# Sbte/RAILS

Measured on AMD Instinct MI355X. Metric: RAILS iterations/sec (+ A*V SpMM HBM GB/s in roofline), m=1M rows/GPU, k=128, fp64, higher is better.
Workload: dtype f64

## Files before the change

include/rails_hip.h:

```cpp
#ifndef RAILS_HIP_H
#define RAILS_HIP_H

#include <stddef.h>
#include <stdint.h>

#ifdef __cplusplus
extern "C" {
#endif

#define RAILS_OK 0
#define RAILS_EINVAL -1
#define RAILS_EHIP -2
#define RAILS_ENOMEM -3
#define RAILS_ELAPACK -4
#define RAILS_ECOMM -5
#define RAILS_ENODEV -6

typedef struct rails_ctx rails_ctx;
typedef struct rails_csr rails_csr;
typedef struct rails_panel rails_panel;

const char *rails_last_error(void);
const char *rails_version(void);

// ... 123 lines not shown
int rails_sweep_plan_array(const rails_sweep_plan *plan, int which, const void **ptr, int64_t *count);


int rails_panel_create(rails_ctx *ctx, int64_t m_local, int capacity, rails_panel **out);
int rails_panel_create_ld(rails_ctx *ctx, int64_t m_local, int capacity, int ld, rails_panel **out);
int rails_panel_destroy(rails_panel *P);
int64_t rails_panel_rows(const rails_panel *P);
int rails_panel_capacity(const rails_panel *P);
int rails_panel_ld(const rails_panel *P);
void *rails_panel_device_ptr(const rails_panel *P);
int rails_panel_reserve(rails_ctx *ctx, rails_panel *P, int capacity);

int rails_panel_upload(rails_ctx *ctx, rails_panel *P, int c0, int nc, const double *host, int64_t ldh);
int rails_panel_download(rails_ctx *ctx, const rails_panel *P, int c0, int nc, double *host, int64_t ldh);

int rails_panel_fill(rails_ctx *ctx, rails_panel *P, int c0, int nc, double value);
int rails_panel_scale(rails_ctx *ctx, rails_panel *P, int c0, int nc, double s);
int rails_panel_copy(rails_ctx *ctx, const rails_panel *X, int xc0, int nc, rails_panel *Y, int yc0);
int rails_panel_axpy(rails_ctx *ctx, double alpha, const rails_panel *X, int xc0, int nc, rails_panel *Y,
                     int yc0);
int rails_panel_random(rails_ctx *ctx, rails_panel *P, int c0, int nc);

int rails_gram(rails_ctx *ctx, const rails_panel *X, int xc0, int a, const rails_panel *Y, int yc0, int b,
               double *C_host, int ldc);

int rails_panel_gemm(rails_ctx *ctx, double alpha, const rails_panel *X, int xc0, int k, const double *C_host,
                     int ldc, int r, double beta, rails_panel *Y, int yc0);

int rails_ctx_enable_library_gemm(rails_ctx *ctx);
int rails_ctx_library_gemm_ready(const rails_ctx *ctx);

int rails_deferred_reserve(rails_ctx *ctx, int nslots, int64_t doubles_per_slot);
int rails_gram_deferred(rails_ctx *ctx, const rails_panel *X, int xc0, int a, const rails_panel *Y, int yc0, int b, int slot);
int rails_panel_gemm_deferred(rails_ctx *ctx, double alpha, const rails_panel *X, int xc0, int k, int slot, int ld, int r, double beta,
                              rails_panel *Y, int yc0);
int rails_chol_inverse_deferred(rails_ctx *ctx, int slot_in, int w, int slot_out);
int rails_update_gram_deferred(rails_ctx *ctx, double alpha, const rails_panel *X, int xc0, int k, const double *C_host, int ldc, int r,
                               rails_panel *Y, int yc0, int r2, int slot);
int rails_update_gram_deferred_out(rails_ctx *ctx, double alpha, const rails_panel *X, int xc0, int k, const double *C_host, int ldc, int r,
                                   const rails_panel *Y, int yc0, rails_panel *Yout, int oc0, int r2, int slot);
int rails_deferred_fetch(rails_ctx *ctx, int slot, int64_t n, double *host_out);

int rails_panel_gemm_wide(rails_ctx *ctx, double alpha, const rails_panel *X, int xc0, int k, const double *C_host, int ldc, int r,
                          double beta, rails_panel *Y, int yc0);

void rails_dense_set_tile_fit(int on);
int rails_dense_tile_fit(void);
int rails_dense_last_tiles(const rails_ctx *ctx, int *update_gram_nbw, int *gram_cols_ti, int *gemm_wide_tr);

void rails_dense_set_update_gram_pipeline(int on);
int rails_dense_update_gram_pipeline(void);
int rails_dense_last_update_gram_form(const rails_ctx *ctx, int *form);

int rails_orthogonalize(rails_ctx *ctx, rails_panel *V, int k_old, int w, int method, int *used);
int rails_orthogonalize_deflated(rails_ctx *ctx, rails_panel *V, int k_old, int w, const rails_panel *N, int nc0, int q, int method, int *used);

int rails_panel_colnorms2(rails_ctx *ctx, const rails_panel *X, int c0, int nc, double *out_host);

int rails_orthogonalize_range(rails_ctx *ctx, rails_panel *V, int k_old, int w, const rails_panel *N, int nc0, int q, double tol, int *kept,
                              int32_t *kept_idx);

int rails_resid_lanczos(rails_ctx *ctx, const rails_panel *AV, int avc0, const rails_panel *MV, int mvc0, int k,
                        const double *T_host, int ldt, const rails_panel *B, int bc0, int p, int L,
                        double *H_host, int ldh, int *steps);

int rails_resid_lanczos_sparse(rails_ctx *ctx, const rails_panel *AV, int avc0, const rails_panel *MV, int mvc0, int k, const double *T_host,
                               int ldt, const rails_sprhs *S, int L, double *H_host, int ldh, int *steps);

int rails_lanczos_start(rails_ctx *ctx, const rails_panel *AV, int avc0, const rails_panel *MV, int mvc0, int k,
                        const rails_panel *B, int bc0, int p, double *sums_host);

int rails_lanczos_vectors(rails_ctx *ctx, const double *S_host, int lds, int w, rails_panel *Out, int oc0);
int rails_lanczos_last_launch(rails_ctx *ctx, int *nch, int *unroll, int *nblocks);
int rails_lanczos_release(rails_ctx *ctx);

int rails_ctx_reserve_staging(rails_ctx *ctx, size_t bytes);
int rails_timer_start(rails_ctx *ctx);
int rails_timer_stop(rails_ctx *ctx, double *ms);


void rails_sb03md(char dico, char job, char fact, char trans, int n, double *A, int lda, double *X, int ldx,
                  double *scale, int *info);
void rails_sb03md_counts(long *smith, long *schur);
void rails_sb03md_adi_counts(long *extended, long *fresh);
void rails_sb03md_set_pause(int calls);
void rails_dsyev(char jobz, char uplo, int n, double *a, int lda, double *w, int *info);
void rails_dsteqr(char compz, int n, double *d, double *e, double *z, int ldz, double *work, int *info);
void rails_dgemm(char transa, char transb, int m, int n, int k, double alpha, const double *A, int lda, const double *B,
                 int ldb, double beta, double *C, int ldc);
void rails_dtrsm(char side, char uplo, char transa, char diag, int m, int n, double alpha, const double *A, int lda, double *B, int ldb);
void rails_dpotrf(char uplo, int n, double *a, int lda, int *info);
void rails_dpstrf(char uplo, int n, double *a, int lda, int *piv, int *rank, double tol, int *info);
void rails_range_basis(int m, int n, double *a, int lda, double tol, double *q, int ldq, int *rank, int *info);
int rails_host_lapack_init(const char *path);
const char *rails_host_lapack_path(void);

#ifdef __cplusplus
}
#endif
#endif
```

rails_amd/_lib.py:

```python
import ctypes as C
import os

_HERE = os.path.dirname(os.path.abspath(__file__))
LIB_PATH = os.path.join(_HERE, "lib", "librails_hip.so")

_dp = C.POINTER(C.c_double)
_ip = C.POINTER(C.c_int)
_i64p = C.POINTER(C.c_int64)
_i32p = C.POINTER(C.c_int32)
_vp = C.c_void_p

ALLREDUCE_FN = C.CFUNCTYPE(C.c_int, C.c_void_p, C.c_void_p, C.c_size_t, C.c_void_p)
HALO_FN = C.CFUNCTYPE(C.c_int, C.c_void_p, C.c_void_p, C.c_void_p, C.c_int, C.c_void_p)
APPLY_FN = C.CFUNCTYPE(C.c_int, C.c_void_p, C.c_int, C.c_void_p, C.c_int, C.c_int, C.c_void_p, C.c_int)

SIGNATURES = {
    "rails_last_error": (C.c_char_p, []),
    "rails_version": (C.c_char_p, []),
    "rails_ctx_create": (C.c_int, [C.c_int, _vp, C.POINTER(_vp)]),
    "rails_ctx_destroy": (C.c_int, [_vp]),
    "rails_ctx_sync": (C.c_int, [_vp]),
    "rails_ctx_stream": (_vp, [_vp]),
    "rails_ctx_num_cu": (C.c_int, [_vp]),
    "rails_ctx_set_meter": (C.c_int, [_vp, C.c_int]),
# ... 53 lines not shown
    "rails_sptrsv_levels": (C.c_int64, [_vp]),
    "rails_sptrsv_solve": (C.c_int, [_vp, _vp, _vp, C.c_int, C.c_int]),
    "rails_panel_permute_rows": (C.c_int, [_vp, _vp, C.c_int, C.c_int, _vp, C.c_int, _vp, C.c_int]),
    "rails_index_upload": (C.c_int, [_vp, _i32p, C.c_int64, C.POINTER(_vp)]),
    "rails_index_free": (None, [_vp, _vp]),
    "rails_lu_create": (C.c_int, [_vp, C.c_int64, _i64p, _i32p, _dp, _i64p, _i32p, _dp, _i32p, _i32p, _i32p, C.c_int64, C.POINTER(_vp)]),
    "rails_lu_destroy": (None, [_vp]),
    "rails_lu_solve": (C.c_int, [_vp, _vp, C.c_int, _vp, C.c_int, C.c_int, _vp, C.c_int]),
    "rails_lu_stats": (C.c_int, [_vp, _i64p, C.c_int]),
    "rails_csr_create_lu": (C.c_int, [_vp, _vp, C.POINTER(_vp)]),
    "rails_iter_create": (C.c_int, [_vp, _vp, C.c_int, _dp, C.POINTER(_vp)]),
    "rails_iter_set": (C.c_int, [_vp, C.c_char_p, C.c_double]),
    "rails_iter_solve": (C.c_int, [_vp, _vp, C.c_int, _vp, C.c_int, C.c_int, _vp, C.c_int]),
    "rails_iter_precondition": (C.c_int, [_vp, _vp, _vp, C.c_int, C.c_int, _vp, C.c_int]),
    "rails_iter_amg_setup": (C.c_int, [_vp, _vp]),
    "rails_iter_amg_info": (C.c_int, [_vp, _i64p, _i64p, _dp, C.c_int]),
    "rails_iter_block_amg_setup": (C.c_int, [_vp, _vp]),
    "rails_iter_block_amg_info": (C.c_int, [_vp, _i64p, _i64p, _dp, C.c_int]),
    "rails_iter_block_jacobi": (C.c_int, [_vp, _vp, C.c_int, _dp]),
    "rails_iter_block_jacobi_info": (C.c_int64, [_vp, _ip, _dp, C.c_int64]),
    "rails_iter_stats": (C.c_int, [_vp, _dp, C.c_int]),
    "rails_iter_columns": (C.c_int, [_vp, _i32p, _dp, _i32p, C.c_int]),
    "rails_csr_create_iter": (C.c_int, [_vp, _vp, C.POINTER(_vp)]),
    "rails_iter_destroy": (None, [_vp]),
    "rails_csr_transpose_host": (C.c_int, [C.c_int64, C.c_int64, _i64p, _i32p, _dp, _i64p, _i32p, _dp]),
    "rails_csr_gram_norm2_host": (C.c_int, [C.c_int64, C.c_int64, _i64p, _i32p, _dp, _i64p, _i32p, _dp, _dp]),
    "rails_bsr_count_host": (C.c_int, [C.c_int64, C.c_int64, C.c_int, _i64p, _i32p, _i64p]),
    "rails_bsr_fill_host": (C.c_int, [C.c_int64, C.c_int64, C.c_int, _i64p, _i32p, _dp, _i64p, _i32p, _dp]),
    "rails_bsr_transpose_host": (C.c_int, [C.c_int64, C.c_int64, C.c_int, _i64p, _i32p, _dp, _i64p, _i32p, _dp]),
    "rails_csr_create_bsr": (C.c_int, [_vp, C.c_int64, C.c_int64, C.c_int, _i64p, _i32p, _dp, C.POINTER(_vp)]),
    "rails_csr_block_size": (C.c_int, [_vp]),
    "rails_csr_bsr_stats": (C.c_int, [_vp, _i64p, C.c_int]),
    "rails_sprhs_create": (C.c_int, [_vp, C.c_int64, C.c_int, _i64p, _i32p, _dp, C.POINTER(_vp)]),
    "rails_sprhs_destroy": (None, [_vp]),
    "rails_sprhs_rows": (C.c_int64, [_vp]),
    "rails_sprhs_cols": (C.c_int64, [_vp]),
    "rails_sprhs_nnz": (C.c_int64, [_vp]),
    "rails_sprhs_gram_norm2": (C.c_double, [_vp]),
    "rails_sprhs_apply": (C.c_int, [_vp, _vp, C.c_int, _vp, C.c_int, C.c_int, _vp, C.c_int]),
    "rails_csr_create_sprhs": (C.c_int, [_vp, _vp, C.POINTER(_vp)]),
    "rails_csr_cols": (C.c_int64, [_vp]),
    "rails_csr_sprhs": (_vp, [_vp]),
    "rails_resid_lanczos_sparse": (C.c_int, [_vp, _vp, C.c_int, _vp, C.c_int, C.c_int, _dp, C.c_int, _vp, C.c_int, _dp, C.c_int, _ip]),
    "rails_panel_random": (C.c_int, [_vp, _vp, C.c_int, C.c_int]),
    "rails_gram": (C.c_int, [_vp, _vp, C.c_int, C.c_int, _vp, C.c_int, C.c_int, _dp, C.c_int]),
    "rails_panel_gemm": (C.c_int, [_vp, C.c_double, _vp, C.c_int, C.c_int, _dp, C.c_int, C.c_int, C.c_double, _vp, C.c_int]),
    "rails_panel_gemm_wide": (C.c_int, [_vp, C.c_double, _vp, C.c_int, C.c_int, _dp, C.c_int, C.c_int, C.c_double, _vp, C.c_int]),
    "rails_dense_set_tile_fit": (None, [C.c_int]),
    "rails_dense_tile_fit": (C.c_int, []),
    "rails_dense_last_tiles": (C.c_int, [_vp, _ip, _ip, _ip]),
    "rails_dense_set_update_gram_pipeline": (None, [C.c_int]),
    "rails_dense_update_gram_pipeline": (C.c_int, []),
    "rails_dense_last_update_gram_form": (C.c_int, [_vp, _ip]),
    "rails_orthogonalize": (C.c_int, [_vp, _vp, C.c_int, C.c_int, C.c_int, _ip]),
    "rails_orthogonalize_deflated": (C.c_int, [_vp, _vp, C.c_int, C.c_int, _vp, C.c_int, C.c_int, C.c_int, _ip]),
    "rails_panel_colnorms2": (C.c_int, [_vp, _vp, C.c_int, C.c_int, _dp]),
    "rails_orthogonalize_range": (C.c_int, [_vp, _vp, C.c_int, C.c_int, _vp, C.c_int, C.c_int, C.c_double, _ip, _i32p]),
    "rails_resid_lanczos": (C.c_int, [_vp, _vp, C.c_int, _vp, C.c_int, C.c_int, _dp, C.c_int, _vp, C.c_int, C.c_int, C.c_int,
                                      _dp, C.c_int, _ip]),
    "rails_lanczos_start": (C.c_int, [_vp, _vp, C.c_int, _vp, C.c_int, C.c_int, _vp, C.c_int, C.c_int, _dp]),
    "rails_lanczos_vectors": (C.c_int, [_vp, _dp, C.c_int, C.c_int, _vp, C.c_int]),
    "rails_lanczos_last_launch": (C.c_int, [_vp, _ip, _ip, _ip]),
    "rails_lanczos_release": (C.c_int, [_vp]),
    "rails_timer_start": (C.c_int, [_vp]),
    "rails_timer_stop": (C.c_int, [_vp, _dp]),
    "rails_sb03md": (None, [C.c_char, C.c_char, C.c_char, C.c_char, C.c_int, _dp, C.c_int, _dp, C.c_int, _dp, _ip]),
    "rails_dsyev": (None, [C.c_char, C.c_char, C.c_int, _dp, C.c_int, _dp, _ip]),
    "rails_dsteqr": (None, [C.c_char, C.c_int, _dp, _dp, _dp, C.c_int, _dp, _ip]),
    "rails_ctx_reserve_staging": (C.c_int, [_vp, C.c_size_t]),
    "rails_sb03md_set_pause": (None, [C.c_int]),
    "rails_sb03md_counts": (None, [C.POINTER(C.c_long), C.POINTER(C.c_long)]),
    "rails_sb03md_adi_counts": (None, [C.POINTER(C.c_long), C.POINTER(C.c_long)]),
    "rails_dtrsm": (None, [C.c_char, C.c_char, C.c_char, C.c_char, C.c_int, C.c_int, C.c_double, _dp, C.c_int, _dp, C.c_int]),
    "rails_dgemm": (None, [C.c_char, C.c_char, C.c_int, C.c_int, C.c_int, C.c_double, _dp, C.c_int, _dp, C.c_int, C.c_double, _dp, C.c_int]),
    "rails_dpotrf": (None, [C.c_char, C.c_int, _dp, C.c_int, _ip]),
    "rails_dpstrf": (None, [C.c_char, C.c_int, _dp, C.c_int, _ip, _ip, C.c_double, _ip]),
    "rails_range_basis": (None, [C.c_int, C.c_int, _dp, C.c_int, C.c_double, _dp, C.c_int, _ip, _ip]),
    "rails_host_lapack_init": (C.c_int, [C.c_char_p]),
    "rails_host_lapack_path": (C.c_char_p, []),
}

_lib = None


class RailsError(RuntimeError):
    pass


def load():
    global _lib
    if _lib is not None:
        return _lib
    if not os.path.exists(LIB_PATH):
        raise RailsError(
            "rails_amd: %s is missing -- build it with `python -c 'import __graft_entry__ as g; g.build()'` "
            "or `make -C rails_amd/csrc`; there is no CPU fallback" % LIB_PATH)
    lib = C.CDLL(LIB_PATH, mode=C.RTLD_GLOBAL)
    for name, (res, args) in SIGNATURES.items():
        fn = getattr(lib, name)
        fn.restype = res
        fn.argtypes = args
    try:
        from ._solver_sigs import bind as _bind_solver
        _bind_solver(lib)
    except ImportError:
        pass
# ... 12 lines not shown
```

rails_amd/csrc/dense_choice.h:

```cpp
#pragma once
#include <algorithm>
#include <cstddef>
#include <cstdint>

namespace dense {

struct DenseSwitches {
    bool tile_fit = true;
    bool update_gram_pipeline = true;
    int gram_cols = 1;
    int gram_extra_column = 1;
    int fused_update_gram = 1;
    int panel_gemm_wide = 1;
    int num_cu = 256;
};

constexpr int inst(int a, int b = 0, int c = 0) { return (a << 16) | (b << 8) | c; }

inline bool rows_vec_ok(const void *ptr, int ld) { return (((uintptr_t)ptr) & 15) == 0 && (ld % 2) == 0; }

#define RAILS_DENSE_GRAM_TABLE(X) X(1, 1) X(8, 1) X(1, 8) X(2, 2) X(4, 2) X(2, 4)
#define RAILS_DENSE_GRAM2_TABLE(X) X(1, 1) X(8, 1) X(4, 2)
#define RAILS_DENSE_GRAM_COLS_TABLE(X) X(4, 1, 0) X(5, 1, 0) X(6, 1, 0) X(4, 1, 1) X(5, 1, 1) X(6, 1, 1) X(3, 2, 0) X(4, 2, 0) X(5, 2, 0)

enum class GramForm { RowSplit, WideX };
struct GramChoice {
    GramForm form;
    int ti, tj, ne;
    int64_t nslab, rps;
    int ngj;
    unsigned grid_y;
    int key() const { return form == GramForm::WideX ? inst(ti, tj, ne) : inst(ti, tj); }
};

inline void gram_slabs(int64_t m, int a, int b, int64_t *nslab_out, int64_t *rps_out)
{
    double bound = 0.02 * (double)m * (double)(a + b) / ((double)a * (double)b);
    int64_t nslab = (int64_t)std::min<double>(1024.0, std::max<double>(1.0, bound));
    int64_t maxslab = (m + 15) / 16;
    if (nslab > maxslab) nslab = std::max<int64_t>(1, maxslab);
    int64_t rps = (m + nslab - 1) / nslab;
    rps = (rps + 15) / 16 * 16;
    if (rps < 16) rps = 16;
    *nslab_out = std::max<int64_t>(1, (m + rps - 1) / rps);
    *rps_out = rps;
}

inline int gram_cols_tiles(int ntiles, bool one_tile, bool tile_fit)
{
    const int cand2[3] = {3, 4, 5}, cand1[3] = {4, 6, 8};
    const int *cand = one_tile ? cand1 : cand2;
    int best = cand[1], best_cost = 1 << 30;
    for (int q = 0; q < 3; ++q) {
        int ti = cand[q], strips = (ntiles + ti - 1) / ti, cost = (strips + 3) / 4 * 4 * ti;
        if (cost < best_cost) best = ti, best_cost = cost;
    }
    if (one_tile && best == 6 && (ntiles + 4) / 5 == (ntiles + 5) / 6 && tile_fit) best = 5;
    return best;
}

inline bool gram_wide_shape(int a, int b) { return b <= 32 && a >= 128; }

inline GramChoice gram_choice(int64_t m, int a, int b, bool two_segment, const DenseSwitches &sw)
{
    GramChoice g{};
    gram_slabs(m, a, b, &g.nslab, &g.rps);
// ... 35 lines not shown
    int64_t ntiles;
    int key() const { return inst(nbw, ne); }
};

inline UpdateGramChoice update_gram_choice(int64_t m, int k, int r, int r2, bool rows_ok, const DenseSwitches &sw)
{
    UpdateGramChoice u{};
    u.fused = sw.fused_update_gram && rows_ok && r <= 17 && r2 <= 16 && k >= 32 && k <= 512 && m >= 4096;
    if (!u.fused) return u;
    u.pipelined = sw.update_gram_pipeline;
    u.ntiles = (m + 15) / 16;
    u.grid = (unsigned)std::min<int64_t>(u.ntiles, 2 * (int64_t)std::max(sw.num_cu, 1));
    u.ne = r > 16 ? 1 : 0;
    if (k <= 256)
        u.nbw = 4;
    else if (k <= 320 && sw.tile_fit)
        u.nbw = 5;
    else if (k <= 384)
        u.nbw = 6;
    else
        u.nbw = 8;
    return u;
}

#define RAILS_DENSE_PANEL_GEMM_TABLE(X) X(1, 32) X(2, 32) X(4, 32) X(8, 32) X(16, 16)
#define RAILS_DENSE_PANEL_GEMM2_TABLE(X) X(1, 32) X(2, 32)

struct PanelGemmChoice {
    int tr, kc;
    int key() const { return inst(tr, kc); }
};

inline PanelGemmChoice panel_gemm_choice(int r)
{
    const int tiles = (r + 15) / 16;
    if (tiles <= 1) return {1, 32};
    if (tiles <= 2) return {2, 32};
    if (tiles <= 4) return {4, 32};
    if (tiles <= 8) return {8, 32};
    return {16, 16};
}
inline PanelGemmChoice panel_gemm2_choice(int r) { return {r <= 16 ? 1 : 2, 32}; }

#define RAILS_DENSE_GEMM_WIDE_TABLE(X) X(6) X(8) X(10) X(12) X(13) X(14) X(15) X(16) X(17) X(18)

struct GemmWideSlice {
    int j0, nc, tr;
};
struct GemmWidePlan {
    bool own_kernel;
    bool tile_fit;
    int r, nslices, width;
    size_t ct_doubles;
    int count() const { return own_kernel ? (r + width - 1) / width : 0; }
    GemmWideSlice slice(int j) const
    {
        const int j0 = j * width, nc = std::min(width, r - j0), exact = (nc + 15) / 16;
        const int tr = (tile_fit && (exact == 13 || exact == 15 || exact == 17)) ? exact : (nc + 31) / 32 * 2;
        return {j0, nc, tr < 6 ? 6 : tr > 18 ? 18 : tr};
    }
};

inline GemmWidePlan gemm_wide_plan(int k, int r, const DenseSwitches &sw)
{
    GemmWidePlan p{};
    p.own_kernel = sw.panel_gemm_wide && r > 64 && k >= 32;
    p.tile_fit = sw.tile_fit;
    p.r = r;
    if (!p.own_kernel) return p;
    p.nslices = (r + 287) / 288;
    p.width = ((r + p.nslices - 1) / p.nslices + 15) / 16 * 16;
    p.ct_doubles = (size_t)((k + 31) / 32 * 32) * (16 * 18 + 4);
    return p;
}

struct Inst {
    int a, b, c;
};
#define RAILS_DENSE_INST2(A, B) {A, B, 0},
#define RAILS_DENSE_INST3(A, B, C) {A, B, C},
#define RAILS_DENSE_INST1(A) {A, 0, 0},
constexpr Inst kGram[] = {RAILS_DENSE_GRAM_TABLE(RAILS_DENSE_INST2)};
constexpr Inst kGram2[] = {RAILS_DENSE_GRAM2_TABLE(RAILS_DENSE_INST2)};
constexpr Inst kGramCols[] = {RAILS_DENSE_GRAM_COLS_TABLE(RAILS_DENSE_INST3)};
constexpr Inst kUpdateGram[] = {RAILS_DENSE_UPDATE_GRAM_TABLE(RAILS_DENSE_INST2)};
constexpr Inst kPanelGemm[] = {RAILS_DENSE_PANEL_GEMM_TABLE(RAILS_DENSE_INST2)};
constexpr Inst kPanelGemm2[] = {RAILS_DENSE_PANEL_GEMM2_TABLE(RAILS_DENSE_INST2)};
constexpr Inst kGemmWide[] = {RAILS_DENSE_GEMM_WIDE_TABLE(RAILS_DENSE_INST1)};
#undef RAILS_DENSE_INST1
#undef RAILS_DENSE_INST2
#undef RAILS_DENSE_INST3

}
```

rails_amd/csrc/dense_common.h:

```cpp
#pragma once
#include "rails_internal.h"

#include <algorithm>
#include <atomic>

#include "dense_choice.h"

struct DenseSwitch {
    const char *variable;
    int on_by_default;
    std::atomic<int> v{-1};
    bool get()
    {
        if (v.load(std::memory_order_relaxed) < 0) {
            const char *e = getenv(variable);
            int undecided = -1;
            v.compare_exchange_strong(undecided, (e ? atoi(e) : on_by_default) ? 1 : 0);
        }
        return v.load(std::memory_order_relaxed) != 0;
    }
    void set(int on) { v.store(on ? 1 : 0); }
};
extern DenseSwitch g_dense_tile_fit;
extern DenseSwitch g_dense_update_gram_pipeline;

int rails_reduce_partials(rails_ctx *c, const double *partial, int64_t nslab, int64_t n, double *out);

inline int upload_coefficients(rails_ctx *c, const double *C_host, int ldc, int k, int r)
{
    const size_t n = (size_t)k * r;
    RAILS_TRY(rails_small_reserve(c, n * sizeof(double)));
    RAILS_TRY(rails_pinned_begin_write(c, n * sizeof(double)));
    for (int j = 0; j < r; ++j) memcpy(c->pinned + (size_t)j * k, C_host + (size_t)j * ldc, sizeof(double) * k);
    RAILS_HIP_CHECK(hipMemcpyAsync(c->small, c->pinned, n * sizeof(double), hipMemcpyHostToDevice, c->stream));
    return rails_pinned_end_write(c);
}

namespace {

typedef double v4f64 __attribute__((ext_vector_type(4)));
typedef double v2f64 __attribute__((ext_vector_type(2)));

__device__ __forceinline__ v4f64 mfma_f64(double a, double b, v4f64 c)
{
    return __builtin_amdgcn_mfma_f64_16x16x4f64(a, b, c, 0, 0, 0);
}

struct OneSeg {
    const double *X;
    int ld;
    struct Row {
        const double *x;
    };
    __device__ int col(int c) const { return c; }
    __device__ Row row(int64_t r) const { return {X + r * ld}; }
    __device__ static const double *at(Row r, int c) { return r.x + c; }
};
struct TwoSeg {
    const double *X1;
    int ld1, a1;
    const double *X2;
    int ld2;
    struct Col {
        int off;
        bool second;
    };
    struct Row {
        const double *x1, *x2;
    };
    __device__ Col col(int c) const
    {
        const bool second = c >= a1;
        return {second ? c - a1 : c, second};
    }
    __device__ Row row(int64_t r) const { return {X1 + r * ld1, X2 + r * ld2}; }
    __device__ static const double *at(Row r, Col c) { return (c.second ? r.x2 : r.x1) + c.off; }
};
// ... 3 lines not shown
```

rails_amd/csrc/dense_gemm.hip:

```cpp
#include "dense_common.h"

#include <dlfcn.h>
#include <mutex>

namespace {

template <int TR, int KC>
__global__ __launch_bounds__(256) void k_panel_gemm(double alpha, const double *X, int ldx, int k,
                                                    const double *__restrict__ C, int r, double beta, double *Yp,
                                                    int ldy, int64_t m, int vec_ok)
{
    const OneSeg Xo{X, ldx};
#define RAILS_PG_VEC4(c) (vec_ok && (c) + 4 <= k)
#include "dense_panel_gemm.inc"
}

template <int TR, int KC>
__global__ __launch_bounds__(256) void k_panel_gemm2(double alpha, const double *X1, int ldx1, int a1, const double *X2, int ldx2, int a,
                                                     const double *__restrict__ C, int r, double beta, double *Yp, int ldy, int64_t m, int vec1,
                                                     int vec2)
{
    const TwoSeg Xo{X1, ldx1, a1, X2, ldx2};
    const int k = a;
#define RAILS_PG_VEC4(c) (((c) + 4 <= a1 && vec1) || ((c) >= a1 && (c) + 4 <= a && vec2))
// ... 52 lines not shown
        }
    };
    double xa[4], xb[4];
    stage(0);
    fetch(4 * kk, xa);
    fetch(16 + 4 * kk, xb);
    asm volatile("s_waitcnt vmcnt(0)" : : : "memory");
    __builtin_amdgcn_s_barrier();
    for (int ci = 0; ci < nchunks; ++ci) {
        if (ci + 1 < nchunks) stage(ci + 1);
        double xc[4], xd[4];
        fetch((ci + 1) * KC + 4 * kk, xc);
        fetch((ci + 1) * KC + 16 + 4 * kk, xd);
        const double *cb = Cs + (size_t)(ci & 1) * (KC * RL);
#pragma unroll
        for (int s = 0; s < 4; ++s) {
            const double *crow = &cb[(4 * kk + s) * RL + li];
#pragma unroll
            for (int t = 0; t < TR; ++t) acc[t] = mfma_f64(xa[s], crow[16 * t], acc[t]);
        }
        if (!skip_tail || ci * KC + 16 < k) {
#pragma unroll
            for (int s = 0; s < 4; ++s) {
                const double *crow = &cb[(16 + 4 * kk + s) * RL + li];
#pragma unroll
                for (int t = 0; t < TR; ++t) acc[t] = mfma_f64(xb[s], crow[16 * t], acc[t]);
            }
        }
#pragma unroll
        for (int s = 0; s < 4; ++s) {
            xa[s] = xc[s];
            xb[s] = xd[s];
        }
        asm volatile("s_waitcnt vmcnt(0) lgkmcnt(0)" : : : "memory");
        __builtin_amdgcn_s_barrier();
    }
#pragma unroll
    for (int t = 0; t < TR; ++t) {
        const int j = 16 * t + li;
        if (j >= r) continue;
#pragma unroll
        for (int v = 0; v < 4; ++v) {
            const int64_t row = r0 + kk + 4 * v;
            if (row >= m) continue;
            double *dst = Yp + row * ldy + j;
            double val = alpha * acc[t][v];
            if (beta != 0.0) val += beta * (*dst);
            *dst = val;
        }
    }
}

template <int TR>
int launch_pg_wide(rails_ctx *c, double alpha, const double *X, int ldx, int k, const double *C, int r, double beta, double *Y, int ldy, int64_t m, int vec_ok, int skip_tail,
                   double *ct)
{
    constexpr int RL = 16 * TR + 4;
    const int kpad = (k + 31) / 32 * 32;
    RAILS_LAUNCH(k_pack_ct, dim3((unsigned)std::min<int64_t>(512, ((int64_t)kpad * RL + 255) / 256)), dim3(256), 0, c->stream, C, k, r, kpad, RL, ct);
    const size_t lds = (size_t)2 * 32 * RL * sizeof(double);
    RAILS_HIP_CHECK(hipFuncSetAttribute((const void *)k_panel_gemm_wide<TR>, hipFuncAttributeMaxDynamicSharedMemorySize, (int)lds));
    RAILS_LAUNCH((k_panel_gemm_wide<TR>), dim3((unsigned)((m + 127) / 128)), dim3(512), lds, c->stream, alpha, X, ldx, k, ct, r, beta, Y, ldy, m, vec_ok,
                 skip_tail);
    c->last_gemm_wide_tr = TR;
    return RAILS_OK;
}

int scale_only(rails_ctx *c, rails_panel *Y, int yc0, int r, double beta)
{
    if (beta == 0.0) return rails_panel_fill(c, Y, yc0, r, 0.0);
    if (beta == 1.0) return RAILS_OK;
    return rails_panel_scale(c, Y, yc0, r, beta);
}

}

int rails_panel_gemm_dev(rails_ctx *c, double alpha, const double *X, int ldx, int k, const double *C_dev, int r, double beta,
                         double *Y, int ldy, int64_t m)
{
    if (r <= 0 || m <= 0) return RAILS_OK;
    const int vec_ok = dense::rows_vec_ok(X, ldx) ? 1 : 0;
    const dense::PanelGemmChoice p = dense::panel_gemm_choice(r);
    const unsigned grid = (unsigned)((m + 63) / 64);
    switch (p.key()) {
#define RAILS_CASE(TR, KC)                                                                                                                 \
    case dense::inst(TR, KC):                                                                                                              \
        RAILS_LAUNCH((k_panel_gemm<TR, KC>), dim3(grid), dim3(256), 0, c->stream, alpha, X, ldx, k, C_dev, r, beta, Y, ldy, m, vec_ok);    \
        break;
        RAILS_DENSE_PANEL_GEMM_TABLE(RAILS_CASE)
#undef RAILS_CASE
    default: RAILS_REQUIRE(false, "rails_panel_gemm: no k_panel_gemm<%d, %d>", p.tr, p.kc);
    }
    RAILS_HIP_CHECK(hipGetLastError());
    return RAILS_OK;
}

int rails_panel_gemm2_dev(rails_ctx *c, double alpha, const double *X1, int ldx1, int a1, const double *X2, int ldx2, int a2, const double *C_dev,
                          int r, double *Y, int ldy, int64_t m)
{
    if (r <= 0 || m <= 0) return RAILS_OK;
    const int a = a1 + a2;
    const int vec1 = dense::rows_vec_ok(X1, ldx1) ? 1 : 0;
    const int vec2 = (dense::rows_vec_ok(X2, ldx2) && (a1 % 2) == 0) ? 1 : 0;
    const dense::PanelGemmChoice p = dense::panel_gemm2_choice(r);
    const unsigned grid = (unsigned)((m + 63) / 64);
    switch (p.key()) {
#define RAILS_CASE(TR, KC)                                                                                                                 \
    case dense::inst(TR, KC):                                                                                                              \
        RAILS_LAUNCH((k_panel_gemm2<TR, KC>), dim3(grid), dim3(256), 0, c->stream, alpha, X1, ldx1, a1, X2, ldx2, a, C_dev, r, 1.0, Y, ldy, m, vec1, vec2); \
        break;
        RAILS_DENSE_PANEL_GEMM2_TABLE(RAILS_CASE)
#undef RAILS_CASE
    default: RAILS_REQUIRE(false, "rails_panel_gemm2: no k_panel_gemm2<%d, %d>", p.tr, p.kc);
    }
    RAILS_HIP_CHECK(hipGetLastError());
    return RAILS_OK;
}
// ... 10 lines not shown
RocblasApi g_rocblas;
std::mutex g_rocblas_mutex;

bool load_rocblas()
{
    std::lock_guard<std::mutex> lock(g_rocblas_mutex);
    if (g_rocblas.tried) return g_rocblas.ok;
    g_rocblas.tried = true;
    const char *e = getenv("RAILS_WIDE_GEMM");
    if (!e || strcmp(e, "rocblas")) return false;
    const char *names[] = {getenv("RAILS_ROCBLAS_LIB"), "librocblas.so", "/opt/rocm/lib/librocblas.so", "librocblas.so.5", "librocblas.so.4"};
    for (const char *n : names) {
        if (!n || !*n) continue;
        if ((g_rocblas.handle = dlopen(n, RTLD_NOW | RTLD_LOCAL))) break;
    }
    if (!g_rocblas.handle) return false;
    g_rocblas.create = (int (*)(void **))dlsym(g_rocblas.handle, "rocblas_create_handle");
    g_rocblas.destroy = (int (*)(void *))dlsym(g_rocblas.handle, "rocblas_destroy_handle");
    g_rocblas.set_stream = (int (*)(void *, hipStream_t))dlsym(g_rocblas.handle, "rocblas_set_stream");
    g_rocblas.dgemm = (decltype(g_rocblas.dgemm))dlsym(g_rocblas.handle, "rocblas_dgemm");
    g_rocblas.ok = g_rocblas.create && g_rocblas.destroy && g_rocblas.set_stream && g_rocblas.dgemm;
    return g_rocblas.ok;
}
constexpr int ROCBLAS_OP_N = 111, ROCBLAS_OP_T = 112;
}

namespace {
struct LibraryGemm {
    std::atomic<int> state{0};
    int device = -1;
    void *handle = nullptr;
    std::mutex use;
};
LibraryGemm g_libgemm;
}

extern "C" int rails_ctx_enable_library_gemm(rails_ctx *c)
{
    RAILS_REQUIRE(c, "rails_ctx_enable_library_gemm: null context");
    std::lock_guard<std::mutex> lock(g_libgemm.use);
    if (g_libgemm.state.load() != 0) return RAILS_OK;
    g_libgemm.device = c->device;
    void *h = nullptr;
    if (!load_rocblas() || hipSetDevice(c->device) != hipSuccess || g_rocblas.create(&h) != 0 || !h) {
        g_libgemm.state = 3;
        return RAILS_OK;
    }
    g_libgemm.handle = h;
    g_libgemm.state = 2;
    return RAILS_OK;
}

extern "C" int rails_ctx_library_gemm_ready(const rails_ctx *c) { return c && g_libgemm.state.load() == 2 && g_libgemm.device == c->device ? 1 : 0; }

extern "C" int rails_panel_gemm_wide(rails_ctx *c, double alpha, const rails_panel *X, int xc0, int k, const double *C_host, int ldc, int r,
                                     double beta, rails_panel *Y, int yc0)
{
    if (c) hipSetDevice(c->device);
    rails_slow_guard slow__(c, "rails_panel_gemm_wide", k, r);
    RAILS_REQUIRE(c && X && Y, "rails_panel_gemm_wide: null argument");
    RAILS_REQUIRE(k >= 0 && r >= 0 && xc0 >= 0 && yc0 >= 0 && xc0 + k <= X->cap && yc0 + r <= Y->cap,
                  "rails_panel_gemm_wide: windows [%d,%d) / [%d,%d) outside capacities %d / %d", xc0, xc0 + k, yc0, yc0 + r, X->cap, Y->cap);
    RAILS_REQUIRE(X->m == Y->m, "rails_panel_gemm_wide: row mismatch %lld vs %lld", (long long)X->m, (long long)Y->m);
    RAILS_REQUIRE(k == 0 || r == 0 || (C_host && ldc >= k), "rails_panel_gemm_wide: bad coefficient matrix (ldc %d < %d)", ldc, k);
    if (X->d == Y->d) RAILS_REQUIRE((xc0 + k <= yc0) || (yc0 + r <= xc0), "rails_panel_gemm_wide: overlapping windows of one panel");
    if (r == 0 || X->m == 0) return RAILS_OK;
    if (k == 0) return scale_only(c, Y, yc0, r, beta);
    RAILS_TRY(upload_coefficients(c, C_host, ldc, k, r));
    if (k >= 64 && r >= 64 && X->m < 0x7fffffffLL && rails_ctx_library_gemm_ready(c)) {
        const int m32 = (int)X->m;
        std::lock_guard<std::mutex> lock(g_libgemm.use);
        int rc = g_rocblas.set_stream(g_libgemm.handle, c->stream);
        if (rc == 0) rc = g_rocblas.dgemm(g_libgemm.handle, ROCBLAS_OP_T, ROCBLAS_OP_N, r, m32, k, &alpha, c->small, k, X->d + xc0, X->ld, &beta, Y->d + yc0, Y->ld);
        if (rc == 0) return RAILS_OK;
        rails_set_error("rails_panel_gemm_wide: rocblas_dgemm failed with status %d", rc);
        return RAILS_EHIP;
    }
    dense::DenseSwitches sw;
    static const int wide_env = spmm_env("RAILS_PANEL_GEMM_WIDE", 1);
    sw.panel_gemm_wide = wide_env;
    sw.tile_fit = g_dense_tile_fit.get();
    const dense::GemmWidePlan plan = dense::gemm_wide_plan(k, r, sw);
    if (!plan.own_kernel) {
        for (int j0 = 0; j0 < r; j0 += 128) {
            const int nc = std::min(128, r - j0);
            RAILS_TRY(rails_panel_gemm_dev(c, alpha, X->d + xc0, X->ld, k, c->small + (size_t)j0 * k, nc, beta, Y->d + yc0 + j0, Y->ld, X->m));
        }
        return RAILS_OK;
    }
    const int vec_ok = dense::rows_vec_ok(X->d + xc0, X->ld) ? 1 : 0;
    RAILS_TRY(rails_ws_reserve(c, (size_t)plan.nslices * plan.ct_doubles * sizeof(double)));
    for (int j = 0; j < plan.count(); ++j) {
        const dense::GemmWideSlice s = plan.slice(j);
        const double *Cj = c->small + (size_t)s.j0 * k;
        double *Yj = Y->d + yc0 + s.j0, *ct = c->ws + (size_t)j * plan.ct_doubles;
        switch (s.tr) {
#define RAILS_CASE(TR)                                                                                                                     \
    case TR:                                                                                                                               \
        RAILS_TRY((launch_pg_wide<TR>(c, alpha, X->d + xc0, X->ld, k, Cj, s.nc, beta, Yj, Y->ld, X->m, vec_ok, plan.tile_fit ? 1 : 0, ct))); \
        break;
            RAILS_DENSE_GEMM_WIDE_TABLE(RAILS_CASE)
#undef RAILS_CASE
        default: RAILS_REQUIRE(false, "rails_panel_gemm_wide: no k_panel_gemm_wide<%d>", s.tr);
        }
    }
    RAILS_HIP_CHECK(hipGetLastError());
    return RAILS_OK;
}

extern "C" int rails_panel_gemm(rails_ctx *c, double alpha, const rails_panel *X, int xc0, int k, const double *C_host, int ldc,
                                int r, double beta, rails_panel *Y, int yc0)
{
    if (c) hipSetDevice(c->device);
    rails_slow_guard slow__(c, "rails_panel_gemm", k, r);
    RAILS_REQUIRE(c && X && Y, "rails_panel_gemm: null argument");
    RAILS_REQUIRE(k >= 0 && r >= 0 && xc0 >= 0 && yc0 >= 0 && xc0 + k <= X->cap && yc0 + r <= Y->cap,
                  "rails_panel_gemm: windows [%d,%d) / [%d,%d) outside capacities %d / %d", xc0, xc0 + k, yc0, yc0 + r, X->cap, Y->cap);
    RAILS_REQUIRE(X->m == Y->m, "rails_panel_gemm: row mismatch %lld vs %lld", (long long)X->m, (long long)Y->m);
    RAILS_REQUIRE(r <= 256, "rails_panel_gemm: r = %d > 256 output columns per call", r);
    RAILS_REQUIRE(k == 0 || r == 0 || (C_host && ldc >= k), "rails_panel_gemm: bad coefficient matrix (ldc %d < %d)", ldc, k);
    if (X->d == Y->d) {
        bool same = (xc0 == yc0);
        bool disjoint = (xc0 + k <= yc0) || (yc0 + r <= xc0);
        RAILS_REQUIRE(same || disjoint, "rails_panel_gemm: partially overlapping windows of one panel");
    }
    if (r == 0 || X->m == 0) return RAILS_OK;
    if (k == 0) return scale_only(c, Y, yc0, r, beta);
    RAILS_TRY(upload_coefficients(c, C_host, ldc, k, r));
    return rails_panel_gemm_dev(c, alpha, X->d + xc0, X->ld, k, c->small, r, beta, Y->d + yc0, Y->ld, X->m);
}
```

rails_amd/csrc/rails_internal.h:

```cpp
#ifndef RAILS_INTERNAL_H
#define RAILS_INTERNAL_H

#include <hip/hip_runtime.h>

#include <cstdarg>
#include <cstdint>
#include <cstdio>
#include <cstring>
#include <ctime>
#include <string>
#include <vector>

#include "rails_hip.h"

void rails_set_error(const char *fmt, ...);

#define RAILS_HIP_CHECK(expr)                                                                      \
    do {                                                                                           \
        hipError_t e__ = (expr);                                                                   \
        if (e__ != hipSuccess) {                                                                   \
            rails_set_error("%s:%d: %s failed: %s", __FILE__, __LINE__, #expr, hipGetErrorString(e__)); \
            return RAILS_EHIP;                                                                     \
        }                                                                                          \
    } while (0)
// ... 3 lines not shown
        if (!(cond)) {                                                                             \
            rails_set_error(__VA_ARGS__);                                                          \
            return RAILS_EINVAL;                                                                   \
        }                                                                                          \
    } while (0)

#define RAILS_TRY(expr)                                                                            \
    do {                                                                                           \
        int rc__ = (expr);                                                                         \
        if (rc__ != RAILS_OK) return rc__;                                                         \
    } while (0)

static inline int rails_pad_ld(int capacity) { return ((capacity < 1 ? 1 : capacity) + 15) / 16 * 16; }

struct rails_ctx {
    int device = 0;
    hipStream_t stream = nullptr;
    bool own_stream = false;
    hipStream_t stream2 = nullptr;
    hipEvent_t ev_fork = nullptr, ev_join = nullptr;
    int num_cu = 256;
    uint64_t seed = 1;
    uint64_t next_stream = 0;
    int rank = 0, nranks = 1;
    int64_t row0 = 0, m_global = -1;
    rails_allreduce_fn allreduce = nullptr;
    void *allreduce_user = nullptr;
    void *rccl = nullptr;
    bool own_rccl = false;
    int rccl_nranks = 0, rccl_rank = 0;
    double *ws = nullptr;
    size_t ws_bytes = 0;
    std::vector<std::pair<size_t, double *>> free_panels;
    size_t free_panel_bytes = 0;
    double *small = nullptr;
    size_t small_bytes = 0;
    double *pinned = nullptr;
    size_t pinned_bytes = 0;
    hipEvent_t ev0 = nullptr, ev1 = nullptr;
    hipEvent_t ev_h2d = nullptr;
    bool h2d_pending = false;
    double *defer_dev = nullptr, *defer_pin = nullptr;
    size_t defer_slot = 0;
    int defer_nslots = 0;
    bool meter = false;
    std::vector<hipEvent_t> meter_events;
    int meter_open = 0;
    long meter_missed = 0;
    double gpu_busy_ms = 0.0;
    void *lz = nullptr;
    long n_orth_block = 0, n_orth_columnwise = 0, n_spmm_tiled = 0, n_spmm_planes = 0, n_spmm_overlapped = 0, n_spmm_sweep = 0, n_spmm_rowgather = 0, n_spmm_callback = 0, n_dev_alloc = 0, n_allreduce = 0, n_lanczos = 0, n_lanczos_start = 0, n_orth_repair = 0, n_update_gram_fused = 0, n_rowquad = 0;
    long n_orth_range = 0, n_orth_range_passes = 0, n_orth_range_syncs = 0;
    int last_update_gram_nbw = 0, last_gram_cols_ti = 0, last_gemm_wide_tr = 0;
    int last_update_gram_form = 0;
    int last_rowquad_nslices = 0, last_rowquad_tr[2] = {0, 0};
};

constexpr int RAILS_METER_PAIRS = 512;
inline bool rails_meter_before(rails_ctx *c)
{
    if (!c->meter) return false;
    if (c->meter_open >= RAILS_METER_PAIRS) {
        c->meter_missed++;
        return false;
    }
    hipEventRecord(c->meter_events[2 * c->meter_open], c->stream);
    return true;
}
inline void rails_meter_after(rails_ctx *c) { hipEventRecord(c->meter_events[2 * c->meter_open++ + 1], c->stream); }
inline hipError_t rails_stream_sync(rails_ctx *c)
{
    const hipError_t e = hipStreamSynchronize(c->stream);
    for (int i = 0; i < c->meter_open; ++i) {
        float ms = 0.0f;
        if (e == hipSuccess && hipEventElapsedTime(&ms, c->meter_events[2 * i], c->meter_events[2 * i + 1]) == hipSuccess) c->gpu_busy_ms += ms;
    }
    c->meter_open = 0;
    return e;
}
#define RAILS_LAUNCH(...)                                                                                                                  \
    do {                                                                                                                                   \
        const bool rails_metered = rails_meter_before(c);                                                                                  \
        hipLaunchKernelGGL(__VA_ARGS__);                                                                                                   \
        if (rails_metered) rails_meter_after(c);                                                                                           \
    } while (0)

struct rails_panel {
    rails_ctx *ctx = nullptr;
    double *d = nullptr;
    int64_t m = 0;
    int cap = 0;
    int ld = 0;
};

struct rails_planes_plan;
struct rails_sweep_cache;
struct rails_tile_cache;
struct rails_bsr;

struct rails_csr {
    rails_ctx *ctx = nullptr;
    rails_sweep_cache *sweep = nullptr;
    rails_planes_plan *planes = nullptr;
    rails_tile_cache *tiled = nullptr;
    int64_t m = 0, ncols_ext = 0, nnz = 0;
    bool rect = false;
// ... 131 lines not shown
```

Measured before the change: 244.9.

## Add persistent grid-stride variant of wide panel GEMM with cross-tile prefetch

Adds a persistent version of the wide panel GEMM kernel that launches at most one workgroup per CU and loops over row tiles. LDS staging of the packed C chunk and the register prefetch of X continue across tile boundaries, so the next tile's loads overlap the current tile's MFMA work and its stores. It targets the launch and tail cost of one workgroup per 128 rows and the pipeline refill at every tile. The form is on by default behind an environment switch. In exchange it re-streams C into LDS for every tile and caps concurrency at one 512-thread workgroup per CU, which may lower the ability to hide memory latency.

```diff
diff --git a/include/rails_hip.h b/include/rails_hip.h
--- a/include/rails_hip.h
+++ b/include/rails_hip.h
@@ -199,6 +199,10 @@
 int rails_dense_update_gram_pipeline(void);
 int rails_dense_last_update_gram_form(const rails_ctx *ctx, int *form);
 
+void rails_dense_set_gemm_wide_persistent(int on);
+int rails_dense_gemm_wide_persistent(void);
+int rails_dense_last_gemm_wide_form(const rails_ctx *ctx, int *form);
+
 int rails_orthogonalize(rails_ctx *ctx, rails_panel *V, int k_old, int w, int method, int *used);
 int rails_orthogonalize_deflated(rails_ctx *ctx, rails_panel *V, int k_old, int w, const rails_panel *N, int nc0, int q, int method, int *used);
 
diff --git a/rails_amd/_lib.py b/rails_amd/_lib.py
--- a/rails_amd/_lib.py
+++ b/rails_amd/_lib.py
@@ -129,6 +129,9 @@
     "rails_dense_set_update_gram_pipeline": (None, [C.c_int]),
     "rails_dense_update_gram_pipeline": (C.c_int, []),
     "rails_dense_last_update_gram_form": (C.c_int, [_vp, _ip]),
+    "rails_dense_set_gemm_wide_persistent": (None, [C.c_int]),
+    "rails_dense_gemm_wide_persistent": (C.c_int, []),
+    "rails_dense_last_gemm_wide_form": (C.c_int, [_vp, _ip]),
     "rails_orthogonalize": (C.c_int, [_vp, _vp, C.c_int, C.c_int, C.c_int, _ip]),
     "rails_orthogonalize_deflated": (C.c_int, [_vp, _vp, C.c_int, C.c_int, _vp, C.c_int, C.c_int, C.c_int, _ip]),
     "rails_panel_colnorms2": (C.c_int, [_vp, _vp, C.c_int, C.c_int, _dp]),
diff --git a/rails_amd/csrc/dense_choice.h b/rails_amd/csrc/dense_choice.h
--- a/rails_amd/csrc/dense_choice.h
+++ b/rails_amd/csrc/dense_choice.h
@@ -12,6 +12,7 @@
     int gram_extra_column = 1;
     int fused_update_gram = 1;
     int panel_gemm_wide = 1;
+    bool gemm_wide_persistent = true;
     int num_cu = 256;
 };
 
@@ -153,6 +154,10 @@
     bool tile_fit;
     int r, nslices, width;
     size_t ct_doubles;
+    bool persistent;
+    int64_t row_tiles;
+    unsigned grid;
+    int64_t tiles_of(unsigned b) const { return b < grid ? (row_tiles - (int64_t)b + grid - 1) / grid : 0; }
     int count() const { return own_kernel ? (r + width - 1) / width : 0; }
     GemmWideSlice slice(int j) const
     {
@@ -172,6 +177,15 @@
     p.nslices = (r + 287) / 288;
     p.width = ((r + p.nslices - 1) / p.nslices + 15) / 16 * 16;
     p.ct_doubles = (size_t)((k + 31) / 32 * 32) * (16 * 18 + 4);
+    return p;
+}
+inline GemmWidePlan gemm_wide_plan(int64_t m, int k, int r, const DenseSwitches &sw)
+{
+    GemmWidePlan p = gemm_wide_plan(k, r, sw);
+    if (!p.own_kernel || m <= 0) return p;
+    p.row_tiles = (m + 127) / 128;
+    p.persistent = sw.gemm_wide_persistent;
+    p.grid = (unsigned)(p.persistent ? std::min<int64_t>(p.row_tiles, (int64_t)std::max(sw.num_cu, 1)) : p.row_tiles);
     return p;
 }
 
diff --git a/rails_amd/csrc/dense_common.h b/rails_amd/csrc/dense_common.h
--- a/rails_amd/csrc/dense_common.h
+++ b/rails_amd/csrc/dense_common.h
@@ -23,6 +23,7 @@
 };
 extern DenseSwitch g_dense_tile_fit;
 extern DenseSwitch g_dense_update_gram_pipeline;
+extern DenseSwitch g_dense_gemm_wide_persistent;
 
 int rails_reduce_partials(rails_ctx *c, const double *partial, int64_t nslab, int64_t n, double *out);
 
diff --git a/rails_amd/csrc/dense_gemm.hip b/rails_amd/csrc/dense_gemm.hip
--- a/rails_amd/csrc/dense_gemm.hip
+++ b/rails_amd/csrc/dense_gemm.hip
@@ -128,17 +128,139 @@
 }
 
 template <int TR>
+__global__ __launch_bounds__(512) void k_panel_gemm_wide_p(double alpha, const double *__restrict__ X, int ldx, int k, const double *__restrict__ Ct ,
+                                                           int r, double beta, double *__restrict__ Yp, int ldy, int64_t m, int vec_ok, int skip_tail)
+{
+    constexpr int KC = 32, RL = 16 * TR + 4, CHUNK_B = KC * RL * 8, PIECES = CHUNK_B / 1024;
+    static_assert(CHUNK_B % 1024 == 0, "whole LDS-DMA pieces per chunk");
+    extern __shared__ double Cs[];
+    const int lane = threadIdx.x & 63;
+    const int wave = __builtin_amdgcn_readfirstlane((int)(threadIdx.x >> 6));
+    const int li = lane & 15, kk = lane >> 4;
+    const int nchunks = (k + KC - 1) / KC;
+    const int64_t ntiles = (m + 127) / 128, grid = gridDim.x;
+    const int64_t nsteps = (ntiles - (int64_t)blockIdx.x + grid - 1) / grid * nchunks;
+    const uint32_t lds_base = (uint32_t)(uintptr_t)(__attribute__((address_space(3))) unsigned char *)Cs;
+    const uint32_t lane16 = (uint32_t)lane * 16u;
+    auto stage = [&](int chunk, int buf) {
+        const char *src = reinterpret_cast<const char *>(Ct) + (size_t)chunk * CHUNK_B;
+        const uint32_t dst = lds_base + (uint32_t)(buf * CHUNK_B);
+        for (int p = wave; p < PIECES; p += 8) {
+            uint32_t keep;
+            asm volatile("s_mov_b32 %0, m0\n\ts_mov_b32 m0, %3\n\ts_nop 0\n\tglobal_load_lds_dwordx4 %1, %2\n\ts_mov_b32 m0, %0"
+                         : "=&s"(keep) : "v"(lane16), "s"(src + (size_t)p * 1024), "s"(dst + (uint32_t)(p * 1024)) : "memory");
+        }
+    };
+    auto rowptr = [&](int64_t tile) {
+        const int64_t row = (tile * 8 + wave) * 16 + li;
+        return X + (row < m ? row : m - 1) * ldx;
+    };
+    auto fetch = [&](const double *xrow, int kcol, double *xs) {
+        if (vec_ok && kcol + 4 <= k) {
+            v2f64 t0 = *reinterpret_cast<const v2f64 *>(xrow + kcol);
+            v2f64 t1 = *reinterpret_cast<const v2f64 *>(xrow + kcol + 2);
+            xs[0] = t0.x;
+            xs[1] = t0.y;
+            xs[2] = t1.x;
+            xs[3] = t1.y;
+        } else {
+#pragma unroll
+            for (int s = 0; s < 4; ++s) xs[s] = (kcol + s < k) ? xrow[kcol + s] : 0.0;
+        }
+    };
+    v4f64 acc[TR];
+#pragma unroll
+    for (int t = 0; t < TR; ++t) acc[t] = (v4f64){0.0, 0.0, 0.0, 0.0};
+    auto store = [&](int64_t tile) {
+        const int64_t r0 = (tile * 8 + wave) * 16;
+#pragma unroll
+        for (int t = 0; t < TR; ++t) {
+            const int j = 16 * t + li;
+            if (j >= r) continue;
+#pragma unroll
+            for (int v = 0; v < 4; ++v) {
+                const int64_t row = r0 + kk + 4 * v;
+                if (row >= m) continue;
+                double *dst = Yp + row * ldy + j;
+                double val = alpha * acc[t][v];
+                if (beta != 0.0) val += beta * (*dst);
+                *dst = val;
+            }
+        }
+    };
+    int64_t tile = blockIdx.x;
+    const double *xrow = rowptr(tile);
+    double xa[4], xb[4];
+    stage(0, 0);
+    fetch(xrow, 4 * kk, xa);
+    fetch(xrow, 16 + 4 * kk, xb);
+    asm volatile("s_waitcnt vmcnt(0)" : : : "memory");
+    __builtin_amdgcn_s_barrier();
+    int ci = 0;
+    for (int64_t step = 0; step < nsteps; ++step) {
+        const bool last_chunk = ci + 1 == nchunks;
+        if (step + 1 < nsteps) stage(last_chunk ? 0 : ci + 1, (int)((step + 1) & 1));
+        const double *xnext = last_chunk ? rowptr(tile + grid) : xrow;
+        const int knext = last_chunk ? 0 : (ci + 1) * KC;
+        double xc[4], xd[4];
+        fetch(xnext, knext + 4 * kk, xc);
+        fetch(xnext, knext + 16 + 4 * kk, xd);
+        if (ci == 0 && step > 0) {
+            store(tile - grid);
+#pragma unroll
+            for (int t = 0; t < TR; ++t) acc[t] = (v4f64){0.0, 0.0, 0.0, 0.0};
+        }
+        const double *cb = Cs + (size_t)(step & 1) * (KC * RL);
+#pragma unroll
+        for (int s = 0; s < 4; ++s) {
+            const double *crow = &cb[(4 * kk + s) * RL + li];
+#pragma unroll
+            for (int t = 0; t < TR; ++t) acc[t] = mfma_f64(xa[s], crow[16 * t], acc[t]);
+        }
+        if (!skip_tail || ci * KC + 16 < k) {
+#pragma unroll
+            for (int s = 0; s < 4; ++s) {
+                const double *crow = &cb[(16 + 4 * kk + s) * RL + li];
+#pragma unroll
+                for (int t = 0; t < TR; ++t) acc[t] = mfma_f64(xb[s], crow[16 * t], acc[t]);
+            }
+        }
+#pragma unroll
+        for (int s = 0; s < 4; ++s) {
+            xa[s] = xc[s];
+            xb[s] = xd[s];
+        }
+        if (last_chunk) {
+            ci = 0;
+            tile += grid;
+            xrow = xnext;
+        } else {
+            ++ci;
+        }
+        asm volatile("s_waitcnt vmcnt(0) lgkmcnt(0)" : : : "memory");
+        __builtin_amdgcn_s_barrier();
+    }
+    store(tile - grid);
+}
+
+template <int TR>
 int launch_pg_wide(rails_ctx *c, double alpha, const double *X, int ldx, int k, const double *C, int r, double beta, double *Y, int ldy, int64_t m, int vec_ok, int skip_tail,
-                   double *ct)
+                   double *ct, bool persistent, unsigned grid)
 {
     constexpr int RL = 16 * TR + 4;
     const int kpad = (k + 31) / 32 * 32;
     RAILS_LAUNCH(k_pack_ct, dim3((unsigned)std::min<int64_t>(512, ((int64_t)kpad * RL + 255) / 256)), dim3(256), 0, c->stream, C, k, r, kpad, RL, ct);
     const size_t lds = (size_t)2 * 32 * RL * sizeof(double);
-    RAILS_HIP_CHECK(hipFuncSetAttribute((const void *)k_panel_gemm_wide<TR>, hipFuncAttributeMaxDynamicSharedMemorySize, (int)lds));
-    RAILS_LAUNCH((k_panel_gemm_wide<TR>), dim3((unsigned)((m + 127) / 128)), dim3(512), lds, c->stream, alpha, X, ldx, k, ct, r, beta, Y, ldy, m, vec_ok,
-                 skip_tail);
+    if (persistent) {
+        RAILS_REQUIRE(grid >= 1 && (int64_t)grid <= (m + 127) / 128, "rails_panel_gemm_wide: %u workgroups for %lld row tiles", grid, (long long)((m + 127) / 128));
+        RAILS_HIP_CHECK(hipFuncSetAttribute((const void *)k_panel_gemm_wide_p<TR>, hipFuncAttributeMaxDynamicSharedMemorySize, (int)lds));
+        RAILS_LAUNCH((k_panel_gemm_wide_p<TR>), dim3(grid), dim3(512), lds, c->stream, alpha, X, ldx, k, ct, r, beta, Y, ldy, m, vec_ok, skip_tail);
+    } else {
+        RAILS_HIP_CHECK(hipFuncSetAttribute((const void *)k_panel_gemm_wide<TR>, hipFuncAttributeMaxDynamicSharedMemorySize, (int)lds));
+        RAILS_LAUNCH((k_panel_gemm_wide<TR>), dim3(grid), dim3(512), lds, c->stream, alpha, X, ldx, k, ct, r, beta, Y, ldy, m, vec_ok, skip_tail);
+    }
     c->last_gemm_wide_tr = TR;
+    c->last_gemm_wide_form = persistent ? 2 : 1;
     return RAILS_OK;
 }
 
@@ -255,6 +377,19 @@
 }
 
 extern "C" int rails_ctx_library_gemm_ready(const rails_ctx *c) { return c && g_libgemm.state.load() == 2 && g_libgemm.device == c->device ? 1 : 0; }
+
+DenseSwitch g_dense_gemm_wide_persistent{"RAILS_GEMM_WIDE_PERSISTENT", 1};
+
+extern "C" void rails_dense_set_gemm_wide_persistent(int on) { g_dense_gemm_wide_persistent.set(on); }
+
+extern "C" int rails_dense_gemm_wide_persistent(void) { return g_dense_gemm_wide_persistent.get() ? 1 : 0; }
+
+extern "C" int rails_dense_last_gemm_wide_form(const rails_ctx *c, int *form)
+{
+    RAILS_REQUIRE(c && form, "rails_dense_last_gemm_wide_form: null argument");
+    *form = c->last_gemm_wide_form;
+    return RAILS_OK;
+}
 
 extern "C" int rails_panel_gemm_wide(rails_ctx *c, double alpha, const rails_panel *X, int xc0, int k, const double *C_host, int ldc, int r,
                                      double beta, rails_panel *Y, int yc0)
@@ -283,7 +418,9 @@
     static const int wide_env = spmm_env("RAILS_PANEL_GEMM_WIDE", 1);
     sw.panel_gemm_wide = wide_env;
     sw.tile_fit = g_dense_tile_fit.get();
-    const dense::GemmWidePlan plan = dense::gemm_wide_plan(k, r, sw);
+    sw.gemm_wide_persistent = g_dense_gemm_wide_persistent.get();
+    sw.num_cu = c->num_cu;
+    const dense::GemmWidePlan plan = dense::gemm_wide_plan(X->m, k, r, sw);
     if (!plan.own_kernel) {
         for (int j0 = 0; j0 < r; j0 += 128) {
             const int nc = std::min(128, r - j0);
@@ -300,7 +437,7 @@
         switch (s.tr) {
 #define RAILS_CASE(TR)                                                                                                                     \
     case TR:                                                                                                                               \
-        RAILS_TRY((launch_pg_wide<TR>(c, alpha, X->d + xc0, X->ld, k, Cj, s.nc, beta, Yj, Y->ld, X->m, vec_ok, plan.tile_fit ? 1 : 0, ct))); \
+        RAILS_TRY((launch_pg_wide<TR>(c, alpha, X->d + xc0, X->ld, k, Cj, s.nc, beta, Yj, Y->ld, X->m, vec_ok, plan.tile_fit ? 1 : 0, ct, plan.persistent, plan.grid))); \
         break;
             RAILS_DENSE_GEMM_WIDE_TABLE(RAILS_CASE)
 #undef RAILS_CASE
diff --git a/rails_amd/csrc/rails_internal.h b/rails_amd/csrc/rails_internal.h
--- a/rails_amd/csrc/rails_internal.h
+++ b/rails_amd/csrc/rails_internal.h
@@ -79,6 +79,7 @@
     long n_orth_block = 0, n_orth_columnwise = 0, n_spmm_tiled = 0, n_spmm_planes = 0, n_spmm_overlapped = 0, n_spmm_sweep = 0, n_spmm_rowgather = 0, n_spmm_callback = 0, n_dev_alloc = 0, n_allreduce = 0, n_lanczos = 0, n_lanczos_start = 0, n_orth_repair = 0, n_update_gram_fused = 0, n_rowquad = 0;
     long n_orth_range = 0, n_orth_range_passes = 0, n_orth_range_syncs = 0;
     int last_update_gram_nbw = 0, last_gram_cols_ti = 0, last_gemm_wide_tr = 0;
+    int last_gemm_wide_form = 0;
     int last_update_gram_form = 0;
     int last_rowquad_nslices = 0, last_rowquad_tr[2] = {0, 0};
 };
```

Result: slower. 242.4 (-1.0%).
